# uwoseis/zephyr

Measured on AMD Instinct MI355X. Metric: wavefields/sec (freq x source solves/s) on 1024^2 grid, higher is better.
Workload: dtype f64

## Files before the change

### zephyr_amd/csrc/nd_factor.hip

```cpp
#include "nd_internal.hpp"
#include <map>
#include <mutex>
#include <cstring>

namespace {

__device__ __forceinline__ long long mf_off(long long off, long long slot, int nf, int kf) { return (long long)nf * off + (long long)kf * slot; }
__device__ __forceinline__ cplx *front_entry(const NdDev &n, cplx *arenaF, cplx *fac, int r, int c, int nf = 1, int kf = 0, int fac_private = 0) {
    const int nmax = n.smax + n.mmax;
    if (r < n.smax) {
        return fac + (fac_private ? n.finv_off : mf_off(n.finv_off, (long long)n.smax * nmax, nf, kf)) + (long long)r * nmax + c;
    }
    return arenaF + mf_off(n.foff, (long long)n.mmax * nmax, nf, kf) + (long long)(r - n.smax) * nmax + c;
}

__global__ __launch_bounds__(256) void k_nd_assemble(const NdDev *nodes, int first, cplx *arenaF, cplx *fac, const cplx *planes, int nz, int nx) {
    const NdDev n = nodes[first + blockIdx.y];
    const long long N = (long long)nz * nx;
    const int tot = n.s + n.m;
    for (int a = blockIdx.x * blockDim.x + threadIdx.x; a < n.smax; a += gridDim.x * blockDim.x)
        if (a >= n.s) *front_entry(n, arenaF, fac, a, a) = cmake(1.0, 0.0);
    for (int a = blockIdx.x * blockDim.x + threadIdx.x; a < tot; a += gridDim.x * blockDim.x) {
        int z, x, ca;
        nd_cell(n, a, z, x, ca);
// ... 468 lines not shown
        NdPlanesSet ps; for (int q2 = 0; q2 < ND_NF_MAX; ++q2) ps.p[q2] = planes;
        HELM_LAUNCH(k_nd_build_front<true>, dim3((nmax + rb - 1) / rb, 1), dim3(256), (size_t)nmax * sizeof(int2), st, f->pd->d_nodes, 0, arenaF, S.lu, ps, P.nz, P.nx, rb,
                           0, n, nf, kf);
        cplx *F21 = arenaF + foff, *F22 = arenaF + foff + g.smax;
        HIP_TRY(op, hipMemcpy2DAsync(S.f21, (size_t)g.smax * sizeof(cplx), F21, (size_t)nmax * sizeof(cplx), (size_t)g.smax * sizeof(cplx), (size_t)g.mmax, hipMemcpyDeviceToDevice, st));
        if (g.smax <= 64) HELM_LAUNCH(k_lu_factor64, dim3(1), dim3(256), 0, st, S.lu, nmax, g.smax, S.piv);
        else HELM_LAUNCH(k_lu_factor, dim3(1), dim3(256), 0, st, S.lu, nmax, g.smax, S.piv);
        HIP_TRY(op, hipMemcpy2DAsync(work, (size_t)g.mmax * sizeof(cplx), S.lu + g.smax, (size_t)nmax * sizeof(cplx), (size_t)g.mmax * sizeof(cplx), (size_t)g.smax, hipMemcpyDeviceToDevice, st));
        HELM_LAUNCH(k_lu_solve, dim3((g.mmax + 15) / 16), dim3(256), 0, st, (const cplx *)S.lu, nmax, g.smax, (const int *)S.piv, work, g.mmax, g.mmax);
        gemm(op, g.mmax, g.mmax, g.smax, mone, S.f21, g.smax, 0, work, g.mmax, 0, one, F22, nmax, 0, 1, nullptr);
        if (getenv("HELM_ND_DEBUG") && atoi(getenv("HELM_ND_DEBUG")) >= 3) {
            auto sum2d = [&](const void *src, size_t pitch, size_t wbytes, size_t rows_) {
                std::vector<unsigned char> h(wbytes * rows_);
                hipMemcpy2D(h.data(), wbytes, src, pitch, wbytes, rows_, hipMemcpyDeviceToHost);
                unsigned long long x = 1469598103934665603ull;
                for (unsigned char c : h) { x ^= c; x *= 1099511628211ull; }
                return x;
            };
            hipStreamSynchronize(st);
            fprintf(stderr, "[helm direct] treated front %d (level %d, s %d of %d, m %d of %d): lu %016llx f12w %016llx piv %016llx f21 %016llx work %016llx f22 %016llx\n", S.node, g.level, n.s, g.smax, n.m, g.mmax,
                    sum2d(S.lu, (size_t)nmax * sizeof(cplx), (size_t)g.smax * sizeof(cplx), g.smax), sum2d(S.lu + g.smax, (size_t)nmax * sizeof(cplx), (size_t)g.mmax * sizeof(cplx), g.smax),
                    sum2d(S.piv, (size_t)g.smax * sizeof(int), (size_t)g.smax * sizeof(int), 1),
                    sum2d(S.f21, (size_t)g.smax * sizeof(cplx), (size_t)g.smax * sizeof(cplx), g.mmax), sum2d(work, (size_t)g.mmax * sizeof(cplx), (size_t)g.mmax * sizeof(cplx), g.smax),
                    sum2d(F22, (size_t)nmax * sizeof(cplx), (size_t)g.mmax * sizeof(cplx), g.mmax));
        }
    }
    const int dbg = getenv("HELM_ND_DEBUG") ? atoi(getenv("HELM_ND_DEBUG")) : 0;
    if (dbg && nflag) fprintf(stderr, "[helm direct] level %d (%s, s = %d, m = %d): %d ill-conditioned front(s) re-eliminated with a pivoted LU\n", g.level, g.leaf ? "leaves" : "separators", g.smax, g.mmax, nflag);
    return check_kernels(op, "re-elimination of ill-conditioned fronts");
}

}

int factor_group_set(helm_op *op, const FacSet &S, size_t gi, cplx *arenaF, cplx *work) {
    NdFactor *f0 = S.f[0];
    const int nf = S.nf;
    const NdPlan &P = f0->pd->plan;
    const NdDev *d_nodes = f0->pd->d_nodes;
    hipStream_t st = op->stream;
    const cplx one = cmake(1, 0), mone = cmake(-1, 0), zero = cmake(0, 0);
    const NdGroup &g = P.groups[gi];
    const int nmax = g.smax + g.mmax;
    const long long fs = (long long)g.mmax * nmax;
    const long long s11 = (long long)g.smax * g.smax, s12 = (long long)g.smax * g.mmax, s1 = (long long)g.smax * nmax;
    const int nbatch = nf * g.cnt;
    cplx *F = arenaF + (long long)nf * g.foff;
    cplx *Finv = f0->d_fac + (long long)nf * g.finv, *G21 = f0->d_fac + (long long)nf * g.g21, *F12 = Finv + g.smax;
    NfDivScope nfdiv(nf);
    const helm_tuning tune = helm_tuning_now();
    const int fused_leaf = tune.nd_fused_leaf;
    const int fused_leaf_min = tune.nd_fused_leaf_min;
    if (fused_leaf && g.leaf && g.cnt >= fused_leaf_min && P.dof == 1 && P.leaf <= 8 && g.smax <= 64 && g.mmax > 0 && g.mmax <= LEAF_MP) {
        const int leaf_dbg = getenv("HELM_LEAF_DBG") ? atoi(getenv("HELM_LEAF_DBG")) : 0;
        for (int k = 0; k < nf; ++k) {
            NdFactor *f = S.f[k];
            if (f->leafflag_elems < (size_t)g.cnt) {
                if (f->d_leafflag) { hipStreamSynchronize(st); helm_pool_free(op->device, f->d_leafflag, f->leafflag_elems * sizeof(int)); f->d_leafflag = nullptr; f->leafflag_elems = 0; }
                int maxcnt = g.cnt;
                for (const NdGroup &q : P.groups) if (q.leaf) maxcnt = std::max(maxcnt, q.cnt);
                f->d_leafflag = (int *)helm_pool_alloc(op->device, (size_t)maxcnt * sizeof(int));
                if (!f->d_leafflag) HELM_FAIL(op, HELM_ERR_DEVICE, "direct solver: allocation of the leaf flags failed");
                f->leafflag_elems = (size_t)maxcnt;
            }
            for (int j0 = 0; j0 < g.cnt; j0 += 65535) {
                const int nb = std::min(65535, g.cnt - j0);
                cplx *g21b = G21 + (long long)j0 * nf * g.mmax * g.smax;
                launch_leaf_factor(st, g.smax, nb, d_nodes, g.first + j0, arenaF, f0->d_fac, g21b, S.planes[k], P.nz, P.nx, f->d_leafflag + j0, leaf_dbg, nf, k);
            }
            f->flops += (double)g.cnt * 8.0 * (2.0 * LEAF_BW * g.smax * (g.smax + g.mmax) + 3.0 * g.mmax * (g.smax + g.mmax));
        }
        return HELM_OK;
    }
    bool schur_gather = false, gather21 = false;
    const bool packs = P.dof <= 2 ? (nmax < (1 << 14) && P.nz < 65536 && P.nx < 32768) : (nmax < 65535 && P.nz < 4096 && P.nx < 4096 && P.dof < 128);
    if ((size_t)nmax * sizeof(int2) <= 64 * 1024 && packs)
        schur_gather = !g.leaf && g.mmax > 0 && P.dof == 1;
    const int stable_smax = 128;
    const bool watch = stable_enabled(P) && !g.leaf && g.mmax > 0 && g.smax <= std::min(stable_smax, LUS_NMAX) && ensure_est(op, f0, std::min(stable_smax, LUS_NMAX)) == HELM_OK;
    double *est = watch ? f0->d_est : nullptr;
    double *est_rows = watch ? est + est_rows_off(P, nf) : nullptr;
    if (schur_gather && tune.nd_fused_sep && g.smax <= 16 && nmax <= 128 && g.cnt >= tune.nd_fused_sep_min && (long long)nbatch <= 0x7fffffffLL &&
        (long long)P.nz * P.nx * 9 * (long long)sizeof(cplx) < (1LL << 32)) {
        NdPlanesSet ps; for (int k = 0; k < ND_NF_MAX; ++k) ps.p[k] = S.planes[k < nf ? k : 0];
        {
            const double sm = (double)g.smax * g.mmax, mm = (double)g.mmax * g.mmax;
            const bool ext = op && op->profiling && tune.prof_ext != 0;
            ExtArm arm(op, ext, 8.0 * (sm * g.smax + mm * g.smax) * nbatch, 16.0 * (2.0 * (double)g.smax * nmax + 2.0 * sm + 1.5 * mm) * nbatch, g.mmax, g.mmax, g.smax, nbatch, 7);
            launch_sep_factor_small(st, g.smax, nbatch, d_nodes, g.first, arenaF, f0->d_fac, G21, ps, P.nz, P.nx, nf, est, est_rows, (long long)nbatch, op->transposed ? 1 : 0);
        }
        if (watch) for (int k = 0; k < nf; ++k) { const int rcf = flag_group(op, S.f[k], gi, est, S.rtol[k]); if (rcf) return rcf; }
        for (int k = 0; k < nf; ++k)
            S.f[k]->flops += (double)g.cnt * 8.0 * (2.0 * g.smax * g.smax * g.smax + (double)g.smax * g.smax * g.mmax + (double)g.smax * g.mmax * g.mmax);
        if (watch) for (int k = 0; k < nf; ++k) { const int rcs = stabilise_group(op, S.f[k], gi, arenaF, work, S.planes[k], est); if (rcs) return rcs; }
        return HELM_OK;
    }
    if ((size_t)nmax * sizeof(int2) <= 64 * 1024 && packs) {
        gather21 = schur_gather && helm_env_int("HELM_ND_GATHER21", 1) != 0 && g.smax <= helm_env_int("HELM_ND_GATHER21_SMAX", ND_GATHER21_SMAX) &&
                   gemm_gather21_ok(op, g.mmax, g.smax, g.smax, nbatch);
        const int brows = gather21 ? g.smax : nmax;
        const int want = std::max(1, 2048 / g.cnt);
        const int rb = std::max(std::min(brows, 4), (brows + want - 1) / want);
        NdPlanesSet ps; for (int k = 0; k < ND_NF_MAX; ++k) ps.p[k] = S.planes[k < nf ? k : 0];
        const int chunk = 65535 / nf;
        for (int j0 = 0; j0 < g.cnt; j0 += chunk) {
            const int nb = std::min(chunk, g.cnt - j0);
            HELM_LAUNCH(k_nd_build_front<false>, dim3((brows + rb - 1) / rb, nb * nf), dim3(256), (size_t)nmax * sizeof(int2), st, d_nodes, g.first + j0, arenaF, f0->d_fac, ps,
                               P.nz, P.nx, rb, gather21 ? 2 : (schur_gather ? 1 : 0), NdDev(), nf, -1);
        }
    } else {
        if (nf != 1) HELM_FAIL(op, HELM_ERR_UNSUPPORTED, "direct solver: fronts of %d unknowns take the unfused build, which factors one frequency at a time", nmax);
        const cplx *planes = S.planes[0];
        if (fs > 0) HIP_TRY(op, hipMemsetAsync(F, 0, (size_t)g.cnt * fs * sizeof(cplx), st));
        HIP_TRY(op, hipMemsetAsync(Finv, 0, (size_t)g.cnt * s1 * sizeof(cplx), st));
        for (int j0 = 0; j0 < g.cnt; j0 += 65535) {
            const int nb = std::min(65535, g.cnt - j0);
            HELM_LAUNCH(k_nd_assemble, dim3((nmax + 255) / 256, nb), dim3(256), 0, st, d_nodes, g.first + j0, arenaF, f0->d_fac, planes, P.nz, P.nx);
        }
        if (!g.leaf) {
            const size_t shm = (size_t)(2 * nmax + 8) * sizeof(int);
            for (int slot = 0; slot < 2; ++slot)
                for (int j0 = 0; j0 < g.cnt; j0 += 65535) {
                    const int nb = std::min(65535, g.cnt - j0);
// ... 123 lines not shown
```

### zephyr_amd/csrc/nd_internal.hpp

```cpp
#pragma once
#include "helm_internal.hpp"
#include "direct.hpp"
#include <hip/hip_ext.h>
#include <algorithm>

struct GjPivotArgs { const cplx *T0; int ld; long long stride; int n, k0, nb; const cplx *Wc0, *Wr0; long long wstride; cplx *Pb0; long long pstride; int batch; };
struct GemmRows {
    const int4 *tabB = nullptr, *tabCi = nullptr, *tabCo = nullptr;
    int offB = 0, offCi = 0, offCo = 0, tab_stride = 0;
    const cplx *Bx = nullptr, *Cix = nullptr; cplx *Cox = nullptr;
    int ldx = 0;
    int z0 = 0;
    int fwd3 = 0;
    int zr0 = 0, zr1 = 0, zc0 = 0, zc1 = 0;
    int sk0 = 0, sk1 = 0;
    int ksplit = 0, kc = 0; long long pstride = 0;
    int dense = 0;
    const cplx *Bx2 = nullptr; int k2 = 0;
    int tm64 = 0;
    const GjPivotArgs *la = nullptr;
    int schur4 = 0;
    const NdDev *nodes = nullptr; int first = 0;
    const cplx *arenaS = nullptr;
    int nf = 1;
// ... 105 lines not shown
            a[i][j] = csub(base, cmul(fcol[i], a[k][j]));
        }
        __syncthreads();
    }
    if (tid < 64) {
        for (int k = n - 1; k >= 0; --k) {
            const int p = piv[k];
            if (p != k && tid < n) { cplx t = a[tid][k]; a[tid][k] = a[tid][p]; a[tid][p] = t; }
        }
    }
    __syncthreads();
}

inline int check_kernels(helm_op *op, const char *what) {
    hipError_t e = hipGetLastError();
    if (e != hipSuccess) { char b[256]; snprintf(b, sizeof(b), "direct solver: %s failed: %s", what, hipGetErrorString(e)); helm_set_error(op, b); return HELM_ERR_DEVICE; }
    return HELM_OK;
}

struct GroupTrace {
    bool on; hipStream_t st; std::vector<hipEvent_t> ev; const char *what;
    GroupTrace(hipStream_t s, const char *w) : st(s), what(w) { const int t = getenv("HELM_ND_TRACE") ? atoi(getenv("HELM_ND_TRACE")) : 0; on = t != 0; mark(); }
    void mark() { if (!on) return; hipEvent_t e; hipEventCreate(&e); hipEventRecord(e, st); ev.push_back(e); }
    void report(const NdPlan &P, bool reverse) {
        if (!on) return;
        hipStreamSynchronize(st);
        double tot = 0;
        for (size_t i = 0; i + 1 < ev.size(); ++i) {
            float ms = 0.f; hipEventElapsedTime(&ms, ev[i], ev[i + 1]); tot += ms;
            const size_t gi = reverse ? P.groups.size() - 1 - i : i;
            if (gi < P.groups.size()) {
                const NdGroup &g = P.groups[gi];
                fprintf(stderr, "[nd trace] %-8s level %2d %s cnt %6d s %5d m %5d : %8.3f ms\n", what, g.level, g.leaf ? "leaf" : "sep ", g.cnt, g.smax, g.mmax, ms);
            } else fprintf(stderr, "[nd trace] %-8s extra : %8.3f ms\n", what, ms);
        }
        fprintf(stderr, "[nd trace] %-8s total %8.3f ms\n", what, tot);
        for (hipEvent_t e : ev) hipEventDestroy(e);
        ev.clear();
    }
};

struct GemmChoice { int tile = 0, kslab = 8, xr = 0, ksplit = 0, kc = 0; };
int gemm(helm_op *op, int M, int Nn, int K, cplx alpha, const cplx *A, int lda, long long sa, const cplx *B, int ldb, long long sb,
         cplx beta, cplx *C, int ldc, long long sc, int batch, const GemmRows *rows = nullptr, GemmChoice *made = nullptr);
bool gemm_gather21_ok(helm_op *op, int M, int Nn, int K, int batch);
extern int g_gemm_tile;
extern int g_gemm_slab;
extern int g_gemm_xcd;
bool gemm_sep_bwd_small(helm_op *op, int smax, int mmax, int nrhs, const cplx *Finv, const cplx *F12, int lda, long long sa, int batch, const GemmRows &rows);
void invert(helm_op *op, cplx *M, int ld, long long stride, int n, int batch, cplx *W, long long ws, int align = 1, int base = 0);
extern int g_recurse_min;
void launch_zgemm3_la(hipStream_t st, bool latency_tile, int nb, int M, int Nn, int K, cplx alpha, const cplx *A, int lda, long long sa, const cplx *B, int ldb, long long sb,
                      cplx beta, cplx *C, int ldc, long long sc, const GemmRows &R, const GjPivotArgs &pv);
void launch_leaf_factor(hipStream_t st, int smax, int nb, const NdDev *d_nodes, int first, cplx *arenaF, cplx *fac, cplx *g21b, const cplx *planes, int nz, int nx, int *flags, int dbg,
                        int nf = 1, int kf = 0);
void launch_sep_factor_small(hipStream_t st, int smax, int nb, const NdDev *d_nodes, int first, cplx *arenaF, cplx *fac, cplx *g21b, const NdPlanesSet &ps, int nz, int nx, int nf,
                             double *est, double *est_rows, long long nbatch_all, int tr);
struct FacSet { int nf = 1; NdFactor *f[ND_NF_MAX] = {nullptr, nullptr, nullptr, nullptr}; const cplx *planes[ND_NF_MAX] = {nullptr, nullptr, nullptr, nullptr}; double rtol[ND_NF_MAX] = {0, 0, 0, 0}; };
int factor_prologue(helm_op *op, int block, NdFactor *f, const cplx *planes_in, const cplx **planes);
int factor_group(helm_op *op, NdFactor *f, size_t gi, cplx *arenaF, cplx *work, const cplx *planes);
bool merged_group(const NdPlan &P, const NdGroup &g);
void launch_lu_solve(hipStream_t st, const cplx *LU, int ld, int n, const int *piv, cplx *B, int ldb, int ncols);
void launch_transpose(hipStream_t st, const cplx *in, long long rows, long long cols, cplx *out, int swap, int conj);
```

### zephyr_amd/csrc/nd_leaf.hip

```cpp
#include "nd_internal.hpp"
#include "nd_gj32w.hpp"

namespace {

#define LEAF_NB 19
#define LEAF_NBR 28
struct LeafTabs {
    int idx[LEAF_MP][3];
    cplx f12[LEAF_MP][3];
    cplx f21[LEAF_MP][3];
};
template <int SP>
__device__ __forceinline__ void leaf_load(const NdDev &n, const cplx *planes, int nz, int nx, cplx *band, float *rowmax, int *brow, LeafTabs &T, int tid, int nthreads) {
    const long long N = (long long)nz * nx;
    const int w = n.x1 - n.x0, h = n.z1 - n.z0;
    for (int e = tid; e < SP * LEAF_NB; e += nthreads) band[e] = (e % LEAF_NB == LEAF_BW && e / LEAF_NB >= n.s) ? cmake(1.0, 0.0) : cmake(0.0, 0.0);
    for (int a = tid; a < SP; a += nthreads) {
        int br = -1;
        if (a < n.s) {
            const int lz = a / w, lx = a % w;
            if (lz == 0 || lz == h - 1 || lx == 0 || lx == w - 1) {
                int cnt = 0;
                for (int q = 0; q < a; ++q) { const int qz = q / w, qx = q % w; if (qz == 0 || qz == h - 1 || qx == 0 || qx == w - 1) cnt += 1; }
                br = cnt;
            }
        }
        brow[a] = br;
        rowmax[a] = 1.0f;
    }
    for (int e = tid; e < LEAF_MP * 3; e += nthreads) { T.idx[e / 3][e % 3] = -1; T.f12[e / 3][e % 3] = cmake(0.0, 0.0); T.f21[e / 3][e % 3] = cmake(0.0, 0.0); }
}
template <int SP>
__device__ __forceinline__ void leaf_fill(const NdDev &n, const cplx *planes, int nz, int nx, cplx *band, float *rowmax, LeafTabs &T, int tid, int nthreads) {
    const long long N = (long long)nz * nx;
    const int w = n.x1 - n.x0;
    for (int a = tid; a < n.s; a += nthreads) {
        const int z = n.z0 + a / w, x = n.x0 + a % w;
        float mx = 0.f;
        #pragma unroll
        for (int k = 0; k < 9; ++k) {
            const int z2 = z + k / 3 - 1, x2 = x + k % 3 - 1;
            if (z2 < n.z0 || z2 >= n.z1 || x2 < n.x0 || x2 >= n.x1) continue;
            const cplx v = planes[(long long)k * N + (long long)z * nx + x];
            const int b = (z2 - n.z0) * w + (x2 - n.x0);
            band[a * LEAF_NB + (b - a) + LEAF_BW] = v;
            mx = fmaxf(mx, (float)fmax(fabs(v.x), fabs(v.y)));
        }
        rowmax[a] = mx;
    }
    for (int r = tid; r < n.m; r += nthreads) {
        int zr, xr;
        nd_cell(n, n.s + r, zr, xr);
        int t = 0;
        for (int k = 0; k < 9; ++k) {
            const int z2 = zr + k / 3 - 1, x2 = xr + k % 3 - 1;
            if (z2 < n.z0 || z2 >= n.z1 || x2 < n.x0 || x2 >= n.x1 || t >= 3) continue;
            const int a = (z2 - n.z0) * w + (x2 - n.x0);
            T.idx[r][t] = a;
            T.f21[r][t] = planes[(long long)k * N + (long long)zr * nx + xr];
            T.f12[r][t] = planes[(long long)(8 - k) * N + (long long)z2 * nx + x2];
            t += 1;
        }
    }
}

template <int SP>
__global__ __launch_bounds__(128, 4) void k_leaf_factor(const NdDev *nodes, int first, cplx *arenaF, cplx *fac, cplx *g21base, const cplx *planes, int nz, int nx, int *flags, int dbg,
                                                        int nf, int kf) {
    __shared__ cplx band[SP * LEAF_NB];
    __shared__ LeafTabs T;
    __shared__ float rowmax[SP];
    __shared__ int brow[SP];
    __shared__ int bad;
    const NdDev n = nodes[first + blockIdx.x];
    const int tid = threadIdx.x;
    const int smax = n.smax, mmax = n.mmax, nmax = smax + mmax;
    if (tid == 0) bad = 0;
    leaf_load<SP>(n, planes, nz, nx, band, rowmax, brow, T, tid, 128);
    __syncthreads();
    leaf_fill<SP>(n, planes, nz, nx, band, rowmax, T, tid, 128);
    __syncthreads();
    if (tid < 64 && !(dbg & 1)) {
        int mybad = 0;
        for (int k = 0; k < SP; ++k) {
            const cplx p = band[k * LEAF_NB + LEAF_BW];
            const double pm = fmax(fabs(p.x), fabs(p.y));
            if (!(pm >= 0.01 * (double)rowmax[k])) mybad = 1;
            const cplx pi = crecip(p);
            for (int e = tid; e < LEAF_BW * LEAF_BW; e += 64) {
                const int di = e / LEAF_BW + 1, dj = e % LEAF_BW + 1;
                const int i = k + di, j = k + dj;
                if (i < SP && j < SP) {
                    const cplx l = cmul(band[i * LEAF_NB + LEAF_BW - di], pi);
                    const cplx u = band[k * LEAF_NB + LEAF_BW + dj];
                    cplx &aij = band[i * LEAF_NB + (j - i) + LEAF_BW];
                    aij = csub(aij, cmul(l, u));
                }
            }
            if (tid < LEAF_BW && k + tid + 1 < SP) { cplx &l = band[(k + tid + 1) * LEAF_NB + LEAF_BW - (tid + 1)]; l = cmul(l, pi); }
            if (tid == LEAF_BW) band[k * LEAF_NB + LEAF_BW] = pi;
        }
        if (mybad && tid == 0) bad = 1;
    }
    __syncthreads();
    if (tid == 0) flags[blockIdx.x] = (dbg & 8) ? 1 : bad;
    const int c = tid;
    const bool active = c < SP + mmax;
    const int gc = c < SP ? c : smax + (c - SP);
    const bool stored = active && (c < SP ? c < smax : true);
    cplx *Fcol = fac + (long long)nf * n.finv_off + (long long)kf * smax * nmax + gc;
    int ra0 = -1, ra1 = -1, ra2 = -1;
    cplx rv0 = cmake(0.0, 0.0), rv1 = rv0, rv2 = rv0;
    if (c < SP) { ra0 = c; rv0 = cmake(1.0, 0.0); }
    else if (c - SP < n.m) {
        ra0 = T.idx[c - SP][0]; rv0 = cneg(T.f12[c - SP][0]);
        ra1 = T.idx[c - SP][1]; rv1 = cneg(T.f12[c - SP][1]);
        ra2 = T.idx[c - SP][2]; rv2 = cneg(T.f12[c - SP][2]);
    }
#define LEAF_RHS(i_) (ra0 == (i_) ? rv0 : (ra1 == (i_) ? rv1 : (ra2 == (i_) ? rv2 : cmake(0.0, 0.0))))
    const int lb = (tid & 63) < LEAF_NB ? (tid & 63) : LEAF_NB - 1;
    auto bcast = [](cplx v, int l) {
        cplx r;
        r.x = __hiloint2double(__builtin_amdgcn_readlane(__double2hiint(v.x), l), __builtin_amdgcn_readlane(__double2loint(v.x), l));
        r.y = __hiloint2double(__builtin_amdgcn_readlane(__double2hiint(v.y), l), __builtin_amdgcn_readlane(__double2loint(v.y), l));
        return r;
    };
    if (!(dbg & 2)) {
        {
            cplx yw[SP];
            cplx cur = band[0 * LEAF_NB + lb];
            #pragma unroll
            for (int i = 0; i < SP; ++i) {
                cplx nxt = cur;
                if (i + 1 < SP) nxt = band[(i + 1) * LEAF_NB + lb];
                cplx acc = LEAF_RHS(i);
                #pragma unroll
                for (int d = 1; d <= LEAF_BW; ++d)
                    if (i - d >= 0) { const cplx l = bcast(cur, LEAF_BW - d); acc.x = fma(l.y, yw[i - d].y, fma(-l.x, yw[i - d].x, acc.x)); acc.y = fma(-l.y, yw[i - d].x, fma(-l.x, yw[i - d].y, acc.y)); }
                yw[i] = acc;
                if (stored && i < smax) Fcol[(long long)i * nmax] = acc;
                cur = nxt;
            }
        }
        {
            constexpr int AHEAD = 6;
            cplx xw[SP], yq[SP];
            #pragma unroll
            for (int i = SP - 1; i >= SP - AHEAD && i >= 0; --i) yq[i] = (stored && i < smax) ? Fcol[(long long)i * nmax] : LEAF_RHS(i);
            cplx cur = band[(SP - 1) * LEAF_NB + lb];
            #pragma unroll
            for (int i = SP - 1; i >= 0; --i) {
                if (i - AHEAD >= 0) yq[i - AHEAD] = (stored && i - AHEAD < smax) ? Fcol[(long long)(i - AHEAD) * nmax] : LEAF_RHS(i - AHEAD);
                cplx nxt = cur;
                if (i > 0) nxt = band[(i - 1) * LEAF_NB + lb];
                cplx acc = yq[i];
                #pragma unroll
                for (int d = 1; d <= LEAF_BW; ++d)
                    if (i + d < SP) { const cplx u = bcast(cur, LEAF_BW + d); acc.x = fma(u.y, xw[i + d].y, fma(-u.x, xw[i + d].x, acc.x)); acc.y = fma(-u.y, xw[i + d].x, fma(-u.x, xw[i + d].y, acc.y)); }
                acc = cmul(acc, bcast(cur, LEAF_BW));
                xw[i] = acc;
                if (stored && i < smax) Fcol[(long long)i * nmax] = acc;
                cur = nxt;
            }
        }
    }
    __syncthreads();
    if (active && !(dbg & 4)) {
        cplx *G21 = g21base + ((long long)blockIdx.x * nf + kf) * mmax * smax;
        cplx *S = arenaF + (long long)nf * n.foff + (long long)kf * mmax * nmax + smax;
        for (int r = 0; r < mmax; ++r) {
            cplx acc = cmake(0.0, 0.0);
            if (r < n.m && stored) {
                #pragma unroll
                for (int t = 0; t < 3; ++t) {
                    const int a = T.idx[r][t];
                    if (a >= 0) cfma(acc, T.f21[r][t], Fcol[(long long)a * nmax]);
                }
            }
            if (c < SP) { if (c < smax) G21[(long long)r * smax + c] = acc; }
            else S[(long long)r * nmax + (c - SP)] = acc;
        }
    }
}


__global__ __launch_bounds__(256) void k_leaf_factor_pivoted(const NdDev *nodes, int first, cplx *arenaF, cplx *fac, cplx *g21base, const cplx *planes, int nz, int nx, const int *flags,
                                                             int nf, int kf) {
    if (!flags[blockIdx.x]) return;
    __shared__ cplx a[GJ_MAX][GJ_MAX + 1];
    __shared__ cplx fcol[GJ_MAX];
    __shared__ int piv[GJ_MAX];
    __shared__ LeafTabs T;
    const NdDev n = nodes[first + blockIdx.x];
    const int tid = threadIdx.x;
    const int smax = n.smax, mmax = n.mmax, nmax = smax + mmax, w = n.x1 - n.x0;
    const long long N = (long long)nz * nx;
    for (int e = tid; e < GJ_MAX * GJ_MAX; e += 256) { const int i = e / GJ_MAX, j = e % GJ_MAX; a[i][j] = (i == j && i >= n.s) ? cmake(1.0, 0.0) : cmake(0.0, 0.0); }
    for (int e = tid; e < LEAF_MP * 3; e += 256) { T.idx[e / 3][e % 3] = -1; T.f12[e / 3][e % 3] = cmake(0.0, 0.0); T.f21[e / 3][e % 3] = cmake(0.0, 0.0); }
    __syncthreads();
    for (int q = tid; q < n.s; q += 256) {
        const int z = n.z0 + q / w, x = n.x0 + q % w;
        for (int k = 0; k < 9; ++k) {
            const int z2 = z + k / 3 - 1, x2 = x + k % 3 - 1;
            if (z2 < n.z0 || z2 >= n.z1 || x2 < n.x0 || x2 >= n.x1) continue;
            a[q][(z2 - n.z0) * w + (x2 - n.x0)] = planes[(long long)k * N + (long long)z * nx + x];
        }
    }
    for (int r = tid; r < n.m; r += 256) {
        int zr, xr;
        nd_cell(n, n.s + r, zr, xr);
        int t = 0;
        for (int k = 0; k < 9; ++k) {
            const int z2 = zr + k / 3 - 1, x2 = xr + k % 3 - 1;
            if (z2 < n.z0 || z2 >= n.z1 || x2 < n.x0 || x2 >= n.x1 || t >= 3) continue;
            T.idx[r][t] = (z2 - n.z0) * w + (x2 - n.x0);
            T.f21[r][t] = planes[(long long)k * N + (long long)zr * nx + xr];
            T.f12[r][t] = planes[(long long)(8 - k) * N + (long long)z2 * nx + x2];
            t += 1;
        }
    }
    __syncthreads();
    gj_lds<GJ_MAX>(a, fcol, piv, smax, tid, 256);
    cplx *Frow = fac + (long long)nf * n.finv_off + (long long)kf * smax * nmax;
    for (int e = tid; e < smax * nmax; e += 256) {
        const int i = e / nmax, cc = e % nmax;
        cplx v;
        if (cc < smax) v = a[i][cc];
        else {
            v = cmake(0.0, 0.0);
            const int b = cc - smax;
            if (b < n.m) for (int t = 0; t < 3; ++t) { const int q = T.idx[b][t]; if (q >= 0) cfma(v, a[i][q], cneg(T.f12[b][t])); }
        }
        Frow[(long long)i * nmax + cc] = v;
    }
    cplx *G21 = g21base + ((long long)blockIdx.x * nf + kf) * mmax * smax;
    cplx *S = arenaF + (long long)nf * n.foff + (long long)kf * mmax * nmax + smax;
    for (int e = tid; e < mmax * nmax; e += 256) {
        const int r = e / nmax, cc = e % nmax;
        cplx v = cmake(0.0, 0.0);
        if (r < n.m) {
            if (cc < smax) { for (int t = 0; t < 3; ++t) { const int q = T.idx[r][t]; if (q >= 0) cfma(v, T.f21[r][t], a[q][cc]); } }
            else {
                const int b = cc - smax;
                if (b < n.m)
                    for (int t = 0; t < 3; ++t) {
                        const int q = T.idx[r][t];
                        if (q < 0) continue;
                        cplx gqb = cmake(0.0, 0.0);
                        for (int u = 0; u < 3; ++u) { const int q2 = T.idx[b][u]; if (q2 >= 0) cfma(gqb, a[q][q2], cneg(T.f12[b][u])); }
                        cfma(v, T.f21[r][t], gqb);
                    }
            }
        }
        if (cc < smax) G21[(long long)r * smax + cc] = v; else S[(long long)r * nmax + (cc - smax)] = v;
    }
}

static __device__ cplx g_sep_zero[4];

template <int AFTER>
__device__ __forceinline__ void sep_cond(const cplx *M, int ld, int n, int tr, double *dsh, unsigned char *lone, double *wsh, double *red, double *out, double *wglob, int tid) {
    const int lane = tid & 63, wv = tid >> 6;
    double best = 0.0;
    if (tr) {
        const int j = tid;
        if (j < n) {
            double v = 0.0, off = 0.0;
            for (int i = 0; i < n; ++i) {
                const cplx a = M[i * ld + j];
                const double m = fabs(a.x) + fabs(a.y);
                v += AFTER ? m * wsh[i] : m;
                if (!AFTER && i != j) off += m;
            }
            if (!AFTER) { dsh[j] = v; lone[j] = off == 0.0; }
            best = v;
        }
        if (AFTER) for (int o = 32; o > 0; o >>= 1) best = fmax(best, __shfl_down(best, o));
    } else
    for (int i = wv; i < n; i += 4) {
        double v = 0.0, off = 0.0;
        for (int j = lane; j < n; j += 64) {
            const cplx a = M[i * ld + j];
            const double m = fabs(a.x) + fabs(a.y);
            v += AFTER ? m * wsh[j] : m;
            if (!AFTER && j != i) off += m;
        }
        for (int o = 32; o > 0; o >>= 1) { v += __shfl_down(v, o); if (!AFTER) off += __shfl_down(off, o); }
        v = __shfl(v, 0);
// ... 163 lines not shown
            const int k = lq + 4 * q;
            if (rok && k < smax) G21[(long long)rr * smax + k] = cmake(gr[q], gi[q]);
        }
        const int4 er = finfo[smax + (rok ? rr : 0)];
        auto load_cv = [&](int cb, cplx (&c0)[4], cplx (&c1)[4]) -> unsigned {
            unsigned mask = 0;
            #pragma unroll
            for (int q = 0; q < 4; ++q) {
                const int c = 16 * cb + lq + 4 * q;
                const bool ok = rok && c < mmax;
                const int4 ec = finfo[smax + (ok ? c : 0)];
                const bool ok0 = ok && er.z >= 0 && ec.z >= 0, ok1 = ok && er.w >= 0 && ec.w >= 0;
                const unsigned o0 = ok0 ? (unsigned)(er.z * ld0 + ec.z) * 16u : 0u, o1 = ok1 ? (unsigned)(er.w * ld1 + ec.w) * 16u : 0u;
                c0[q] = at(S0, o0);
                c1[q] = at(S1, o1);
                mask |= (ok0 ? 1u : 0u) << q | (ok1 ? 16u : 0u) << q;
            }
            return mask;
        };
        for (int cb = 0; cb < nblk; ++cb) {
            cplx nx0[4], nx1[4];
            const unsigned nmask = load_cv(cb, nx0, nx1);
            v4f64 sr = (v4f64){0, 0, 0, 0}, si = (v4f64){0, 0, 0, 0};
            #pragma unroll
            for (int g = 0; g < KG; ++g) {
                const int k = 4 * g + lq, cc = 16 * cb + lr;
                const bool in = k < smax && cc < mmax;
                cplx fb = FS[in ? k * nmax + smax + cc : 0];
                if (!in) fb = cmake(0.0, 0.0);
                const double ar = gr[g], ai = gi[g];
                sr = __builtin_amdgcn_mfma_f64_16x16x4f64(fb.x, ar, sr, 0, 0, 0);
                si = __builtin_amdgcn_mfma_f64_16x16x4f64(fb.y, ar, si, 0, 0, 0);
                sr = __builtin_amdgcn_mfma_f64_16x16x4f64(fb.y, -ai, sr, 0, 0, 0);
                si = __builtin_amdgcn_mfma_f64_16x16x4f64(fb.x, ai, si, 0, 0, 0);
            }
            #pragma unroll
            for (int q = 0; q < 4; ++q) {
                const int c = 16 * cb + lq + 4 * q;
                const cplx cv = cadd((nmask >> q) & 1u ? nx0[q] : cmake(0.0, 0.0), (nmask >> (4 + q)) & 1u ? nx1[q] : cmake(0.0, 0.0));
                if (rok && c < mmax) S[(long long)rr * nmax + c] = cadd(cv, cmul(mone, cmake(sr[q], si[q])));
            }
        }
    }
}

}

void launch_sep_factor_small(hipStream_t st, int smax, int nb, const NdDev *d_nodes, int first, cplx *arenaF, cplx *fac, cplx *g21b, const NdPlanesSet &ps, int nz, int nx, int nf,
                             double *est, double *est_rows, long long nbatch_all, int tr) {
    if (smax <= 8) ZG_LAUNCH(k_sep_factor_small<8>, dim3(nb), d_nodes, first, arenaF, fac, g21b, ps, nz, nx, nf, est, est_rows, nbatch_all, tr);
    else ZG_LAUNCH(k_sep_factor_small<16>, dim3(nb), d_nodes, first, arenaF, fac, g21b, ps, nz, nx, nf, est, est_rows, nbatch_all, tr);
}

void launch_leaf_factor(hipStream_t st, int smax, int nb, const NdDev *d_nodes, int first, cplx *arenaF, cplx *fac, cplx *g21b, const cplx *planes, int nz, int nx, int *flags, int dbg,
                        int nf, int kf) {
    if (smax <= 49) HELM_LAUNCH(k_leaf_factor<49>, dim3(nb), dim3(128), 0, st, d_nodes, first, arenaF, fac, g21b, planes, nz, nx, flags, dbg, nf, kf);
    else HELM_LAUNCH(k_leaf_factor<64>, dim3(nb), dim3(128), 0, st, d_nodes, first, arenaF, fac, g21b, planes, nz, nx, flags, dbg, nf, kf);
    HELM_LAUNCH(k_leaf_factor_pivoted, dim3(nb), dim3(256), 0, st, d_nodes, first, arenaF, fac, g21b, planes, nz, nx, (const int *)flags, nf, kf);
}
```

Baseline: 16370.

## Batch leaf factorisation across frequencies with single-wave leaf kernel

Leaf factorisation now runs as one launch covering every leaf and frequency pair, with the block index decoded into leaf and frequency. The old per-frequency loop of launches is gone and leaf flags live in one shared buffer. The 128-thread leaf kernel is replaced by a 64-thread single-wave kernel. Its solve is a compile-time unrolled recursive forward/backward sweep that builds the F12 columns on the fly through an LDS row, and the G21/S products are computed in register-blocked row chunks. This aims to cut launch overhead and idle threads, at the cost of heavier register pressure from the fully unrolled SP-length arrays, plus a new optional debug host readback.

```diff
diff --git a/zephyr_amd/csrc/nd_factor.hip b/zephyr_amd/csrc/nd_factor.hip
--- a/zephyr_amd/csrc/nd_factor.hip
+++ b/zephyr_amd/csrc/nd_factor.hip
@@ -544,22 +544,29 @@
     const int fused_leaf_min = tune.nd_fused_leaf_min;
     if (fused_leaf && g.leaf && g.cnt >= fused_leaf_min && P.dof == 1 && P.leaf <= 8 && g.smax <= 64 && g.mmax > 0 && g.mmax <= LEAF_MP) {
         const int leaf_dbg = getenv("HELM_LEAF_DBG") ? atoi(getenv("HELM_LEAF_DBG")) : 0;
-        for (int k = 0; k < nf; ++k) {
-            NdFactor *f = S.f[k];
-            if (f->leafflag_elems < (size_t)g.cnt) {
-                if (f->d_leafflag) { hipStreamSynchronize(st); helm_pool_free(op->device, f->d_leafflag, f->leafflag_elems * sizeof(int)); f->d_leafflag = nullptr; f->leafflag_elems = 0; }
-                int maxcnt = g.cnt;
-                for (const NdGroup &q : P.groups) if (q.leaf) maxcnt = std::max(maxcnt, q.cnt);
-                f->d_leafflag = (int *)helm_pool_alloc(op->device, (size_t)maxcnt * sizeof(int));
-                if (!f->d_leafflag) HELM_FAIL(op, HELM_ERR_DEVICE, "direct solver: allocation of the leaf flags failed");
-                f->leafflag_elems = (size_t)maxcnt;
-            }
-            for (int j0 = 0; j0 < g.cnt; j0 += 65535) {
-                const int nb = std::min(65535, g.cnt - j0);
-                cplx *g21b = G21 + (long long)j0 * nf * g.mmax * g.smax;
-                launch_leaf_factor(st, g.smax, nb, d_nodes, g.first + j0, arenaF, f0->d_fac, g21b, S.planes[k], P.nz, P.nx, f->d_leafflag + j0, leaf_dbg, nf, k);
-            }
-            f->flops += (double)g.cnt * 8.0 * (2.0 * LEAF_BW * g.smax * (g.smax + g.mmax) + 3.0 * g.mmax * (g.smax + g.mmax));
+        if (f0->leafflag_elems < (size_t)g.cnt * nf) {
+            if (f0->d_leafflag) { hipStreamSynchronize(st); helm_pool_free(op->device, f0->d_leafflag, f0->leafflag_elems * sizeof(int)); f0->d_leafflag = nullptr; f0->leafflag_elems = 0; }
+            int maxcnt = g.cnt;
+            for (const NdGroup &q : P.groups) if (q.leaf) maxcnt = std::max(maxcnt, q.cnt);
+            f0->d_leafflag = (int *)helm_pool_alloc(op->device, (size_t)maxcnt * nf * sizeof(int));
+            if (!f0->d_leafflag) HELM_FAIL(op, HELM_ERR_DEVICE, "direct solver: allocation of the leaf flags failed");
+            f0->leafflag_elems = (size_t)maxcnt * nf;
+        }
+        NdPlanesSet ps; for (int k = 0; k < ND_NF_MAX; ++k) ps.p[k] = S.planes[k < nf ? k : 0];
+        const int chunk = 65535 / nf;
+        for (int j0 = 0; j0 < g.cnt; j0 += chunk) {
+            const int nb = std::min(chunk, g.cnt - j0);
+            cplx *g21b = G21 + (long long)j0 * nf * g.mmax * g.smax;
+            launch_leaf_factor(st, g.smax, nb * nf, d_nodes, g.first + j0, arenaF, f0->d_fac, g21b, ps, P.nz, P.nx, f0->d_leafflag + (size_t)j0 * nf, leaf_dbg, nf);
+        }
+        for (int k = 0; k < nf; ++k) S.f[k]->flops += (double)g.cnt * 8.0 * (2.0 * LEAF_BW * g.smax * (g.smax + g.mmax) + 3.0 * g.mmax * (g.smax + g.mmax));
+        if (getenv("HELM_ND_DEBUG") && atoi(getenv("HELM_ND_DEBUG")) >= 1) {
+            std::vector<int> h((size_t)g.cnt * nf);
+            hipStreamSynchronize(st);
+            hipMemcpy(h.data(), f0->d_leafflag, h.size() * sizeof(int), hipMemcpyDeviceToHost);
+            int nflag = 0;
+            for (int v : h) nflag += v != 0;
+            if (nflag) fprintf(stderr, "[helm direct] level %d (leaves, s = %d, m = %d): %d of %d leaf factorisation(s) re-done with row pivoting\n", g.level, g.smax, g.mmax, nflag, nbatch);
         }
         return HELM_OK;
     }
diff --git a/zephyr_amd/csrc/nd_internal.hpp b/zephyr_amd/csrc/nd_internal.hpp
--- a/zephyr_amd/csrc/nd_internal.hpp
+++ b/zephyr_amd/csrc/nd_internal.hpp
@@ -181,8 +181,8 @@
 extern int g_recurse_min;
 void launch_zgemm3_la(hipStream_t st, bool latency_tile, int nb, int M, int Nn, int K, cplx alpha, const cplx *A, int lda, long long sa, const cplx *B, int ldb, long long sb,
                       cplx beta, cplx *C, int ldc, long long sc, const GemmRows &R, const GjPivotArgs &pv);
-void launch_leaf_factor(hipStream_t st, int smax, int nb, const NdDev *d_nodes, int first, cplx *arenaF, cplx *fac, cplx *g21b, const cplx *planes, int nz, int nx, int *flags, int dbg,
-                        int nf = 1, int kf = 0);
+void launch_leaf_factor(hipStream_t st, int smax, int nb, const NdDev *d_nodes, int first, cplx *arenaF, cplx *fac, cplx *g21b, const NdPlanesSet &ps, int nz, int nx, int *flags, int dbg,
+                        int nf);
 void launch_sep_factor_small(hipStream_t st, int smax, int nb, const NdDev *d_nodes, int first, cplx *arenaF, cplx *fac, cplx *g21b, const NdPlanesSet &ps, int nz, int nx, int nf,
                              double *est, double *est_rows, long long nbatch_all, int tr);
 struct FacSet { int nf = 1; NdFactor *f[ND_NF_MAX] = {nullptr, nullptr, nullptr, nullptr}; const cplx *planes[ND_NF_MAX] = {nullptr, nullptr, nullptr, nullptr}; double rtol[ND_NF_MAX] = {0, 0, 0, 0}; };
diff --git a/zephyr_amd/csrc/nd_leaf.hip b/zephyr_amd/csrc/nd_leaf.hip
--- a/zephyr_amd/csrc/nd_leaf.hip
+++ b/zephyr_amd/csrc/nd_leaf.hip
@@ -4,30 +4,15 @@
 namespace {
 
 #define LEAF_NB 19
-#define LEAF_NBR 28
 struct LeafTabs {
     int idx[LEAF_MP][3];
     cplx f12[LEAF_MP][3];
     cplx f21[LEAF_MP][3];
 };
 template <int SP>
-__device__ __forceinline__ void leaf_load(const NdDev &n, const cplx *planes, int nz, int nx, cplx *band, float *rowmax, int *brow, LeafTabs &T, int tid, int nthreads) {
-    const long long N = (long long)nz * nx;
-    const int w = n.x1 - n.x0, h = n.z1 - n.z0;
+__device__ __forceinline__ void leaf_load(const NdDev &n, cplx *band, float *rowmax, LeafTabs &T, int tid, int nthreads) {
     for (int e = tid; e < SP * LEAF_NB; e += nthreads) band[e] = (e % LEAF_NB == LEAF_BW && e / LEAF_NB >= n.s) ? cmake(1.0, 0.0) : cmake(0.0, 0.0);
-    for (int a = tid; a < SP; a += nthreads) {
-        int br = -1;
-        if (a < n.s) {
-            const int lz = a / w, lx = a % w;
-            if (lz == 0 || lz == h - 1 || lx == 0 || lx == w - 1) {
-                int cnt = 0;
-                for (int q = 0; q < a; ++q) { const int qz = q / w, qx = q % w; if (qz == 0 || qz == h - 1 || qx == 0 || qx == w - 1) cnt += 1; }
-                br = cnt;
-            }
-        }
-        brow[a] = br;
-        rowmax[a] = 1.0f;
-    }
+    for (int a = tid; a < SP; a += nthreads) rowmax[a] = 1.0f;
     for (int e = tid; e < LEAF_MP * 3; e += nthreads) { T.idx[e / 3][e % 3] = -1; T.f12[e / 3][e % 3] = cmake(0.0, 0.0); T.f21[e / 3][e % 3] = cmake(0.0, 0.0); }
 }
 template <int SP>
@@ -64,134 +49,154 @@
     }
 }
 
-template <int SP>
-__global__ __launch_bounds__(128, 4) void k_leaf_factor(const NdDev *nodes, int first, cplx *arenaF, cplx *fac, cplx *g21base, const cplx *planes, int nz, int nx, int *flags, int dbg,
-                                                        int nf, int kf) {
+struct LeafSweep {
+    const cplx *band; cplx *xrow; const LeafTabs *T; cplx *Frow;
+    int lb, c, smax, mmax, nmax, ga0, ga1, ga2;
+    bool gcol;
+};
+__device__ __forceinline__ cplx leaf_bcast(cplx v, int l) {
+    cplx r;
+    r.x = __hiloint2double(__builtin_amdgcn_readlane(__double2hiint(v.x), l), __builtin_amdgcn_readlane(__double2loint(v.x), l));
+    r.y = __hiloint2double(__builtin_amdgcn_readlane(__double2hiint(v.y), l), __builtin_amdgcn_readlane(__double2loint(v.y), l));
+    return r;
+}
+template <int SP, int I>
+__device__ __forceinline__ void leaf_fwd_rows(cplx (&x)[SP], cplx cur, const LeafSweep &w) {
+    cplx nxt = cur;
+    if (I + 1 < SP) nxt = w.band[(I + 1 < SP ? I + 1 : I) * LEAF_NB + w.lb];
+    cplx acc = cmake(w.c == I ? 1.0 : 0.0, 0.0);
+    #pragma unroll
+    for (int d = 1; d <= LEAF_BW; ++d)
+        if (I - d >= 0) {
+            const cplx l = leaf_bcast(cur, LEAF_BW - d), y = x[I - d >= 0 ? I - d : 0];
+            acc.x = fma(l.y, y.y, fma(-l.x, y.x, acc.x)); acc.y = fma(-l.y, y.x, fma(-l.x, y.y, acc.y));
+        }
+    x[I] = acc;
+    if constexpr (I + 1 < SP) leaf_fwd_rows<SP, I + 1>(x, nxt, w);
+}
+template <int SP, int I>
+__device__ __forceinline__ void leaf_bwd_rows(cplx (&x)[SP], cplx cur, const LeafSweep &w) {
+    cplx nxt = cur;
+    if (I > 0) nxt = w.band[(I > 0 ? I - 1 : 0) * LEAF_NB + w.lb];
+    cplx acc = x[I];
+    #pragma unroll
+    for (int d = 1; d <= LEAF_BW; ++d)
+        if (I + d < SP) {
+            const cplx u = leaf_bcast(cur, LEAF_BW + d), xv = x[I + d < SP ? I + d : I];
+            acc.x = fma(u.y, xv.y, fma(-u.x, xv.x, acc.x)); acc.y = fma(-u.y, xv.x, fma(-u.x, xv.y, acc.y));
+        }
+    acc = cmul(acc, leaf_bcast(cur, LEAF_BW));
+    x[I] = acc;
+    if (I < w.smax) {
+        const int c = w.c;
+        cplx *row = w.Frow + (long long)I * w.nmax;
+        if (c < w.smax) row[c] = acc;
+        if (c < SP) w.xrow[c] = acc;
+        __builtin_amdgcn_wave_barrier();
+        if (c < w.mmax) {
+            cplx v = cmake(0.0, 0.0);
+            if (w.gcol) { cfma(v, w.xrow[w.ga0], cneg(w.T->f12[c][0])); cfma(v, w.xrow[w.ga1], cneg(w.T->f12[c][1])); cfma(v, w.xrow[w.ga2], cneg(w.T->f12[c][2])); }
+            row[w.smax + c] = v;
+        }
+        __builtin_amdgcn_wave_barrier();
+    }
+    if constexpr (I > 0) leaf_bwd_rows<SP, I - 1>(x, nxt, w);
+}
+
+template <int SP, int WPS>
+__global__ __launch_bounds__(64, WPS) void k_leaf_wave(const NdDev *nodes, int first, cplx *arenaF, cplx *fac, cplx *g21base, NdPlanesSet pset, int nz, int nx, int *flags, int dbg, int nf) {
     __shared__ cplx band[SP * LEAF_NB];
     __shared__ LeafTabs T;
     __shared__ float rowmax[SP];
-    __shared__ int brow[SP];
-    __shared__ int bad;
-    const NdDev n = nodes[first + blockIdx.x];
+    __shared__ cplx xrow[SP];
+    const long long b = blockIdx.x;
+    const int leaf = (int)(b / nf), kf = (int)(b - (long long)leaf * nf);
+    const cplx *planes = pset.p[kf];
+    const NdDev n = nodes[first + leaf];
     const int tid = threadIdx.x;
     const int smax = n.smax, mmax = n.mmax, nmax = smax + mmax;
-    if (tid == 0) bad = 0;
-    leaf_load<SP>(n, planes, nz, nx, band, rowmax, brow, T, tid, 128);
-    __syncthreads();
-    leaf_fill<SP>(n, planes, nz, nx, band, rowmax, T, tid, 128);
-    __syncthreads();
-    if (tid < 64 && !(dbg & 1)) {
-        int mybad = 0;
-        for (int k = 0; k < SP; ++k) {
-            const cplx p = band[k * LEAF_NB + LEAF_BW];
-            const double pm = fmax(fabs(p.x), fabs(p.y));
-            if (!(pm >= 0.01 * (double)rowmax[k])) mybad = 1;
-            const cplx pi = crecip(p);
-            for (int e = tid; e < LEAF_BW * LEAF_BW; e += 64) {
-                const int di = e / LEAF_BW + 1, dj = e % LEAF_BW + 1;
-                const int i = k + di, j = k + dj;
-                if (i < SP && j < SP) {
-                    const cplx l = cmul(band[i * LEAF_NB + LEAF_BW - di], pi);
-                    const cplx u = band[k * LEAF_NB + LEAF_BW + dj];
-                    cplx &aij = band[i * LEAF_NB + (j - i) + LEAF_BW];
-                    aij = csub(aij, cmul(l, u));
-                }
-            }
-            if (tid < LEAF_BW && k + tid + 1 < SP) { cplx &l = band[(k + tid + 1) * LEAF_NB + LEAF_BW - (tid + 1)]; l = cmul(l, pi); }
-            if (tid == LEAF_BW) band[k * LEAF_NB + LEAF_BW] = pi;
-        }
-        if (mybad && tid == 0) bad = 1;
-    }
-    __syncthreads();
-    if (tid == 0) flags[blockIdx.x] = (dbg & 8) ? 1 : bad;
+    leaf_load<SP>(n, band, rowmax, T, tid, 64);
+    __syncthreads();
+    leaf_fill<SP>(n, planes, nz, nx, band, rowmax, T, tid, 64);
+    __syncthreads();
+    int bad = 0;
+    for (int k = 0; k < ((dbg & 1) ? 0 : SP); ++k) {
+        const cplx p = band[k * LEAF_NB + LEAF_BW];
+        const double pm = fmax(fabs(p.x), fabs(p.y));
+        if (!(pm >= 0.01 * (double)rowmax[k])) bad = 1;
+        const cplx pi = crecip(p);
+        for (int e = tid; e < LEAF_BW * LEAF_BW; e += 64) {
+            const int di = e / LEAF_BW + 1, dj = e % LEAF_BW + 1;
+            const int i = k + di, j = k + dj;
+            if (i < SP && j < SP) {
+                const cplx l = cmul(band[i * LEAF_NB + LEAF_BW - di], pi);
+                const cplx u = band[k * LEAF_NB + LEAF_BW + dj];
+                cplx &aij = band[i * LEAF_NB + (j - i) + LEAF_BW];
+                aij = csub(aij, cmul(l, u));
+            }
+        }
+        if (tid < LEAF_BW && k + tid + 1 < SP) { cplx &l = band[(k + tid + 1) * LEAF_NB + LEAF_BW - (tid + 1)]; l = cmul(l, pi); }
+        if (tid == LEAF_BW) band[k * LEAF_NB + LEAF_BW] = pi;
+    }
+    __syncthreads();
+    if (tid == 0) flags[b] = (dbg & 8) ? 1 : bad;
+    cplx *Frow = fac + (long long)nf * n.finv_off + (long long)kf * smax * nmax;
     const int c = tid;
-    const bool active = c < SP + mmax;
-    const int gc = c < SP ? c : smax + (c - SP);
-    const bool stored = active && (c < SP ? c < smax : true);
-    cplx *Fcol = fac + (long long)nf * n.finv_off + (long long)kf * smax * nmax + gc;
-    int ra0 = -1, ra1 = -1, ra2 = -1;
-    cplx rv0 = cmake(0.0, 0.0), rv1 = rv0, rv2 = rv0;
-    if (c < SP) { ra0 = c; rv0 = cmake(1.0, 0.0); }
-    else if (c - SP < n.m) {
-        ra0 = T.idx[c - SP][0]; rv0 = cneg(T.f12[c - SP][0]);
-        ra1 = T.idx[c - SP][1]; rv1 = cneg(T.f12[c - SP][1]);
-        ra2 = T.idx[c - SP][2]; rv2 = cneg(T.f12[c - SP][2]);
-    }
-#define LEAF_RHS(i_) (ra0 == (i_) ? rv0 : (ra1 == (i_) ? rv1 : (ra2 == (i_) ? rv2 : cmake(0.0, 0.0))))
-    const int lb = (tid & 63) < LEAF_NB ? (tid & 63) : LEAF_NB - 1;
-    auto bcast = [](cplx v, int l) {
-        cplx r;
-        r.x = __hiloint2double(__builtin_amdgcn_readlane(__double2hiint(v.x), l), __builtin_amdgcn_readlane(__double2loint(v.x), l));
-        r.y = __hiloint2double(__builtin_amdgcn_readlane(__double2hiint(v.y), l), __builtin_amdgcn_readlane(__double2loint(v.y), l));
-        return r;
-    };
+    const int lb = tid < LEAF_NB ? tid : LEAF_NB - 1;
+    int ga0 = 0, ga1 = 0, ga2 = 0;
+    const bool gcol = c < n.m;
+    if (gcol) { ga0 = max(T.idx[c][0], 0); ga1 = max(T.idx[c][1], 0); ga2 = max(T.idx[c][2], 0); }
+    cplx x[SP];
+    const LeafSweep w = {band, xrow, &T, Frow, lb, c, smax, mmax, nmax, ga0, ga1, ga2, gcol};
     if (!(dbg & 2)) {
-        {
-            cplx yw[SP];
-            cplx cur = band[0 * LEAF_NB + lb];
+    leaf_fwd_rows<SP, 0>(x, band[0 * LEAF_NB + lb], w);
+    leaf_bwd_rows<SP, SP - 1>(x, band[(SP - 1) * LEAF_NB + lb], w);
+    }
+    __syncthreads();
+    if (dbg & 4) return;
+    cplx *G21 = g21base + b * mmax * smax;
+    cplx *S = arenaF + (long long)nf * n.foff + (long long)kf * mmax * nmax + smax;
+    const bool on1 = c < smax, on2 = c < mmax;
+    const cplx *X1 = Frow + (on1 ? c : 0), *X2 = Frow + smax + (on2 ? c : 0);
+    constexpr int RB = 8;
+    for (int r0 = 0; r0 < mmax; r0 += RB) {
+        cplx v1[RB][3], v2[RB][3];
+        #pragma unroll
+        for (int u = 0; u < RB; ++u) {
+            const int r = min(r0 + u, LEAF_MP - 1);
             #pragma unroll
-            for (int i = 0; i < SP; ++i) {
-                cplx nxt = cur;
-                if (i + 1 < SP) nxt = band[(i + 1) * LEAF_NB + lb];
-                cplx acc = LEAF_RHS(i);
-                #pragma unroll
-                for (int d = 1; d <= LEAF_BW; ++d)
-                    if (i - d >= 0) { const cplx l = bcast(cur, LEAF_BW - d); acc.x = fma(l.y, yw[i - d].y, fma(-l.x, yw[i - d].x, acc.x)); acc.y = fma(-l.y, yw[i - d].x, fma(-l.x, yw[i - d].y, acc.y)); }
-                yw[i] = acc;
-                if (stored && i < smax) Fcol[(long long)i * nmax] = acc;
-                cur = nxt;
-            }
-        }
-        {
-            constexpr int AHEAD = 6;
-            cplx xw[SP], yq[SP];
+            for (int t = 0; t < 3; ++t) {
+                const long long o = (long long)max(T.idx[r][t], 0) * nmax;
+                v1[u][t] = X1[o];
+                v2[u][t] = X2[o];
+            }
+        }
+        #pragma unroll
+        for (int u = 0; u < RB; ++u) {
+            const int r = r0 + u, rr = min(r, LEAF_MP - 1);
+            cplx a1 = cmake(0.0, 0.0), a2 = cmake(0.0, 0.0);
             #pragma unroll
-            for (int i = SP - 1; i >= SP - AHEAD && i >= 0; --i) yq[i] = (stored && i < smax) ? Fcol[(long long)i * nmax] : LEAF_RHS(i);
-            cplx cur = band[(SP - 1) * LEAF_NB + lb];
-            #pragma unroll
-            for (int i = SP - 1; i >= 0; --i) {
-                if (i - AHEAD >= 0) yq[i - AHEAD] = (stored && i - AHEAD < smax) ? Fcol[(long long)(i - AHEAD) * nmax] : LEAF_RHS(i - AHEAD);
-                cplx nxt = cur;
-                if (i > 0) nxt = band[(i - 1) * LEAF_NB + lb];
-                cplx acc = yq[i];
-                #pragma unroll
-                for (int d = 1; d <= LEAF_BW; ++d)
-                    if (i + d < SP) { const cplx u = bcast(cur, LEAF_BW + d); acc.x = fma(u.y, xw[i + d].y, fma(-u.x, xw[i + d].x, acc.x)); acc.y = fma(-u.y, xw[i + d].x, fma(-u.x, xw[i + d].y, acc.y)); }
-                acc = cmul(acc, bcast(cur, LEAF_BW));
-                xw[i] = acc;
-                if (stored && i < smax) Fcol[(long long)i * nmax] = acc;
-                cur = nxt;
-            }
-        }
-    }
-    __syncthreads();
-    if (active && !(dbg & 4)) {
-        cplx *G21 = g21base + ((long long)blockIdx.x * nf + kf) * mmax * smax;
-        cplx *S = arenaF + (long long)nf * n.foff + (long long)kf * mmax * nmax + smax;
-        for (int r = 0; r < mmax; ++r) {
-            cplx acc = cmake(0.0, 0.0);
-            if (r < n.m && stored) {
-                #pragma unroll
-                for (int t = 0; t < 3; ++t) {
-                    const int a = T.idx[r][t];
-                    if (a >= 0) cfma(acc, T.f21[r][t], Fcol[(long long)a * nmax]);
-                }
-            }
-            if (c < SP) { if (c < smax) G21[(long long)r * smax + c] = acc; }
-            else S[(long long)r * nmax + (c - SP)] = acc;
-        }
-    }
-}
-
-
-__global__ __launch_bounds__(256) void k_leaf_factor_pivoted(const NdDev *nodes, int first, cplx *arenaF, cplx *fac, cplx *g21base, const cplx *planes, int nz, int nx, const int *flags,
-                                                             int nf, int kf) {
+            for (int t = 0; t < 3; ++t) { const cplx f = T.f21[rr][t]; cfma(a1, f, v1[u][t]); cfma(a2, f, v2[u][t]); }
+            if (r < mmax) {
+                if (on1) G21[(long long)r * smax + c] = a1;
+                if (on2) S[(long long)r * nmax + c] = a2;
+            }
+        }
+    }
+}
+
+
+__global__ __launch_bounds__(256) void k_leaf_factor_pivoted(const NdDev *nodes, int first, cplx *arenaF, cplx *fac, cplx *g21base, NdPlanesSet pset, int nz, int nx, const int *flags,
+                                                             int nf) {
     if (!flags[blockIdx.x]) return;
+    const long long b = blockIdx.x;
+    const int leaf = (int)(b / nf), kf = (int)(b - (long long)leaf * nf);
+    const cplx *planes = pset.p[kf];
     __shared__ cplx a[GJ_MAX][GJ_MAX + 1];
     __shared__ cplx fcol[GJ_MAX];
     __shared__ int piv[GJ_MAX];
     __shared__ LeafTabs T;
-    const NdDev n = nodes[first + blockIdx.x];
+    const NdDev n = nodes[first + leaf];
     const int tid = threadIdx.x;
     const int smax = n.smax, mmax = n.mmax, nmax = smax + mmax, w = n.x1 - n.x0;
     const long long N = (long long)nz * nx;
@@ -233,7 +238,7 @@
         }
         Frow[(long long)i * nmax + cc] = v;
     }
-    cplx *G21 = g21base + ((long long)blockIdx.x * nf + kf) * mmax * smax;
+    cplx *G21 = g21base + b * mmax * smax;
     cplx *S = arenaF + (long long)nf * n.foff + (long long)kf * mmax * nmax + smax;
     for (int e = tid; e < mmax * nmax; e += 256) {
         const int r = e / nmax, cc = e % nmax;
@@ -503,9 +508,9 @@
     else ZG_LAUNCH(k_sep_factor_small<16>, dim3(nb), d_nodes, first, arenaF, fac, g21b, ps, nz, nx, nf, est, est_rows, nbatch_all, tr);
 }
 
-void launch_leaf_factor(hipStream_t st, int smax, int nb, const NdDev *d_nodes, int first, cplx *arenaF, cplx *fac, cplx *g21b, const cplx *planes, int nz, int nx, int *flags, int dbg,
-                        int nf, int kf) {
-    if (smax <= 49) HELM_LAUNCH(k_leaf_factor<49>, dim3(nb), dim3(128), 0, st, d_nodes, first, arenaF, fac, g21b, planes, nz, nx, flags, dbg, nf, kf);
-    else HELM_LAUNCH(k_leaf_factor<64>, dim3(nb), dim3(128), 0, st, d_nodes, first, arenaF, fac, g21b, planes, nz, nx, flags, dbg, nf, kf);
-    HELM_LAUNCH(k_leaf_factor_pivoted, dim3(nb), dim3(256), 0, st, d_nodes, first, arenaF, fac, g21b, planes, nz, nx, (const int *)flags, nf, kf);
-}
+void launch_leaf_factor(hipStream_t st, int smax, int nb, const NdDev *d_nodes, int first, cplx *arenaF, cplx *fac, cplx *g21b, const NdPlanesSet &ps, int nz, int nx, int *flags, int dbg,
+                        int nf) {
+    if (smax <= 49) HELM_LAUNCH((k_leaf_wave<49, 2>), dim3(nb), dim3(64), 0, st, d_nodes, first, arenaF, fac, g21b, ps, nz, nx, flags, dbg, nf);
+    else HELM_LAUNCH((k_leaf_wave<64, 1>), dim3(nb), dim3(64), 0, st, d_nodes, first, arenaF, fac, g21b, ps, nz, nx, flags, dbg, nf);
+    HELM_LAUNCH(k_leaf_factor_pivoted, dim3(nb), dim3(256), 0, st, d_nodes, first, arenaF, fac, g21b, ps, nz, nx, (const int *)flags, nf);
+}
```

New measurement: 15150. -7.4%, worse.
